# kivicode/TensorHive-Fixed

Hardware: AMD Instinct MI355X
Metric: llama3_8b_bf16_ddp_train_tokens_per_sec (higher is better)
Workload: dtype bf16; 1 GPU; model=Llama-3-8B, global_batch=8, micro_batch=8, grad_accum=1, seq_len=4096, parallelism=dp1, optimizer=AdamW (fp32 master, fused flat kernel, clip 1.0), zero=0, attention=hip, gemm_table=True, gemm_table_kind=gemm_gfx950_t32768.csv

## Files before the change

### tensorhive_fixed_amd/ops/csrc/flash_attn.hip

```cpp
#include "th_common.h"

typedef __bf16 bf16x8 __attribute__((ext_vector_type(8)));
typedef float f32x16 __attribute__((ext_vector_type(16)));
typedef short i16x4 __attribute__((ext_vector_type(4)));
#define LDS_AS __attribute__((address_space(3)))

namespace {
constexpr int HD = 128;
constexpr float LOG2E = 1.4426950408889634f;
constexpr float LN2 = 0.6931471805599453f;

__device__ __forceinline__ int img_off(int row, int ch) {
  return ((row >> 3) << 11) + ((ch >> 2) << 9) + ((row & 7) << 6) + (((ch & 3) ^ ((row >> 2) & 3)) << 4);
}

__device__ __forceinline__ bf16x8 as_bf(ushort8 u) { return __builtin_bit_cast(bf16x8, u); }

__device__ __forceinline__ bf16x8 lds_row(const char* img, int row, int ch) {
  return *reinterpret_cast<const bf16x8*>(img + img_off(row, ch));
}

__device__ __forceinline__ bf16x8 lds_tr(const char* img, int rbase, int cbase, int lane) {
  const int h = lane >> 5, grp = (lane >> 4) & 1, i = lane & 15;
  const int row = rbase + 4 * h + (i >> 2);
  const int col = cbase + 16 * grp + 4 * (i & 3);
  const char* p0 = img + img_off(row, col >> 3) + ((col & 7) << 1);
  const char* p1 = img + img_off(row + 8, col >> 3) + ((col & 7) << 1);
  const i16x4 lo = __builtin_amdgcn_ds_read_tr16_b64_v4i16((LDS_AS i16x4*)(p0));
  const i16x4 hi = __builtin_amdgcn_ds_read_tr16_b64_v4i16((LDS_AS i16x4*)(p1));
  typedef short i16x8 __attribute__((ext_vector_type(8)));
  const i16x8 v = {lo[0], lo[1], lo[2], lo[3], hi[0], hi[1], hi[2], hi[3]};
  return __builtin_bit_cast(bf16x8, v);
}

#ifndef TH_FA_PRIO
#define TH_FA_PRIO 1
#endif
#define FA_PRIO(p)                                  \
  do {                                              \
    if (TH_FA_PRIO) __builtin_amdgcn_s_setprio(p); \
  } while (0)

__device__ __forceinline__ f32x16 mfma(bf16x8 a, bf16x8 b, f32x16 c) {
  return __builtin_amdgcn_mfma_f32_32x32x16_bf16(a, b, c, 0, 0, 0);
}

__device__ __forceinline__ bf16x8 pack8(const f32x16& x, int base) {
  bf16x8 r;
#pragma unroll
  for (int j = 0; j < 8; ++j) r[j] = (__bf16)x[base + j];
  return r;
}

__device__ __forceinline__ void store_row_t21(ushort* row, const f32x16 (&acc)[4], float f, int h) {
#pragma unroll
  for (int d = 0; d < 4; ++d)
#pragma unroll
    for (int p = 0; p < 2; ++p) {
      unsigned a[2], c[2];
#pragma unroll
      for (int k = 0; k < 2; ++k) {
        a[k] = (unsigned)f2bf(acc[d][8 * p + 2 * k] * f) | ((unsigned)f2bf(acc[d][8 * p + 2 * k + 1] * f) << 16);
        c[k] = (unsigned)f2bf(acc[d][8 * p + 4 + 2 * k] * f) | ((unsigned)f2bf(acc[d][8 * p + 5 + 2 * k] * f) << 16);
        const auto r = __builtin_amdgcn_permlane32_swap(a[k], c[k], false, false);
        a[k] = r[0];
        c[k] = r[1];
      }
      typedef unsigned u32x4 __attribute__((ext_vector_type(4)));
      const u32x4 v = {a[0], a[1], c[0], c[1]};
      *reinterpret_cast<u32x4*>(row + 32 * d + 16 * p + 8 * h) = v;
    }
}

__device__ __forceinline__ void rope_bwd_rows(f32x16 (&a)[4], const float* __restrict__ rcos,
                                              const float* __restrict__ rsin, int pos, int h) {
  const float* cr = rcos + (long)pos * 64;
  const float* sr = rsin + (long)pos * 64;
#pragma unroll
  for (int d = 0; d < 2; ++d)
#pragma unroll
    for (int g = 0; g < 4; ++g) {
      const float4v c4 = *reinterpret_cast<const float4v*>(cr + 32 * d + 8 * g + 4 * h);
      const float4v s4 = *reinterpret_cast<const float4v*>(sr + 32 * d + 8 * g + 4 * h);
#pragma unroll
      for (int e = 0; e < 4; ++e) {
        const float x = a[d][4 * g + e], y = a[d + 2][4 * g + e];
        a[d][4 * g + e] = x * c4[e] + y * s4[e];
        a[d + 2][4 * g + e] = y * c4[e] - x * s4[e];
      }
    }
}

__device__ __forceinline__ int xcd_remap(int bid, int nwg) {
  const int xcd = bid & 7, q = nwg >> 3, r = nwg & 7;
  return (xcd < r ? xcd * (q + 1) : r * (q + 1) + (xcd - r) * q) + (bid >> 3);
}

__device__ __forceinline__ int acc_row(int r, int h) { return (r & 3) + 8 * (r >> 2) + 4 * h; }

__device__ __forceinline__ int stage_row(int tid) { return 2 * ((tid >> 3) & 7) + ((tid >> 2) & 1); }
__device__ __forceinline__ int stage_ch(int tid) { return 4 * ((tid >> 6) & 3) + (tid & 3); }
template <int NP>
__device__ __forceinline__ void stage_load(ushort8 (&r)[NP], const ushort* base, long ld, int row0,
                                           int limit, int tid) {
#pragma unroll
  for (int i = 0; i < NP; ++i) {
    const int row = min(row0 + 16 * i + stage_row(tid), limit - 1);
    r[i] = *reinterpret_cast<const ushort8*>(base + (long)row * ld + (stage_ch(tid) << 3));
  }
}
template <int NP>
__device__ __forceinline__ void stage_store(char* img, const ushort8 (&r)[NP], int tid) {
#pragma unroll
  for (int i = 0; i < NP; ++i)
    *reinterpret_cast<ushort8*>(img + img_off(16 * i + stage_row(tid), stage_ch(tid))) = r[i];
}

template <bool KVMAJOR>
__device__ __forceinline__ void q_block_map(int L, int nqb, int B, int Hq, int Hkv, int& b, int& hq, int& qb) {
  if (KVMAJOR) {
    const int G = Hq / Hkv, per = nqb * G;
    const int grp = L / per, r = L % per;
    b = grp / Hkv;
    hq = (grp % Hkv) * G + r % G;
    qb = nqb - 1 - r / G;
  } else {
    const int per = Hq * B;
    qb = nqb - 1 - L / per;
    const int rem = L % per;
    b = rem / Hq;
    hq = rem % Hq;
  }
}

__device__ __forceinline__ void glds16(const void* sbase, unsigned voff, unsigned lds) {
  asm volatile("s_mov_b32 m0, %0\n\ts_nop 0\n\tglobal_load_lds_dwordx4 %1, %2"
               :: "s"(lds), "v"(voff), "s"(sbase) : "memory", "m0");
}
__device__ __forceinline__ void glds4(const void* sbase, unsigned voff, unsigned lds) {
  asm volatile("s_mov_b32 m0, %0\n\ts_nop 0\n\tglobal_load_lds_dword %1, %2"
               :: "s"(lds), "v"(voff), "s"(sbase) : "memory", "m0");
}
__device__ __forceinline__ unsigned img_rc(unsigned o) {
  const unsigned row = ((o >> 11) << 3) | ((o >> 6) & 7);
  const unsigned ch = (((o >> 9) & 3) << 2) | (((o >> 4) & 3) ^ ((row >> 2) & 3));
  return row | (ch << 8);
}
__device__ __forceinline__ void wait_dma_barrier() { asm volatile("s_waitcnt vmcnt(0)\n\ts_barrier" ::: "memory"); }
__device__ __forceinline__ void dma_kv_tile(const ushort* Kb, const ushort* Vb, long ld, int S, int jt, unsigned lds0,
                                            int wu, const unsigned (&rc)[4]) {
  const unsigned img = lds0 + (jt & 1) * (2 * 64 * 256) + wu * 4096;
#pragma unroll
  for (int u = 0; u < 4; ++u) {
    const int row = min(jt * 64 + (int)(rc[u] & 255), S - 1);
    const unsigned voff = (unsigned)(row * ld + (rc[u] >> 8) * 8) * 2u;
    glds16(Kb, voff, img + u * 1024);
    glds16(Vb, voff, img + 64 * 256 + u * 1024);
  }
}

__device__ __forceinline__ void dma_kv_piece(const ushort* Kb, const ushort* Vb, long ld, int S, int jt,
                                             unsigned lds0, int wu, const unsigned (&rc)[4], int p) {
  const unsigned img = lds0 + (jt & 1) * (2 * 64 * 256) + wu * 4096;
  const int u = p >> 1;
  const int row = min(jt * 64 + (int)(rc[u] & 255), S - 1);
  const unsigned voff = (unsigned)(row * ld + (rc[u] >> 8) * 8) * 2u;
  if (p & 1)
    glds16(Vb, voff, img + 64 * 256 + u * 1024);
  else
    glds16(Kb, voff, img + u * 1024);
}

#ifndef TH_FA_FWD_SPREAD
#define TH_FA_FWD_SPREAD 0
#endif
#ifndef TH_FA_FWD_DEFAULT
#define TH_FA_FWD_DEFAULT 15
#endif
// ... 218 lines not shown
          if (ks4 == 2) {
            pf[2] = pack8(sacc[1], 0);
            pf[3] = pack8(sacc[1], 8);
          }
          bf16x8 nx[4];
#pragma unroll
          for (int d = 0; d < 4; ++d) nx[d] = ks4 < 3 ? lds_tr(vs, 16 * ks4 + 16, 32 * d, lane) : vt[d];
          __builtin_amdgcn_sched_barrier(0);
#pragma unroll
          for (int d = 0; d < 4; ++d) {
            o[d] = mfma(vt[d], pf[ks4], o[d]);
            if (ks4 < 2) {
              p_of(1, 8 * ks4 + 2 * d);
              p_of(1, 8 * ks4 + 2 * d + 1);
            }
          }
          __builtin_amdgcn_sched_barrier(0);
#pragma unroll
          for (int d = 0; d < 4; ++d) vt[d] = nx[d];
        }
        FA_PRIO(0);
      }
      const float rs = (rs4[0] + rs4[1]) + (rs4[2] + rs4[3]);
      l_i += half_swap_sum(rs);
    }
  }

  if (q < S) {
    const float inv_l = l_i > 0.f ? 1.f / l_i : 0.f;
    store_row_t21(O + b * bso + (long)q * ldo + (long)hq * HD, o, inv_l, h);
    if (h == 0) LSE[((long)b * Hq + hq) * S + q] = (m_i + log2f(l_i)) * LN2;
  }
}

#ifdef TH_FA_DIAG
constexpr int PP_R = 4, PP_SLOT = 2 * F_BN * 256;
#ifndef TH_PP_PRIO
#define TH_PP_PRIO 0
#endif
#ifndef TH_PP_SHIFT
#define TH_PP_SHIFT 0
#endif
#ifndef TH_PP_NMF
#define TH_PP_NMF 0
#endif
#ifndef TH_PP_YPRIO
#define TH_PP_YPRIO 0
#endif
#ifdef TH_PP_STAMP
constexpr int PP_STAMP_STEPS = 72;
__device__ unsigned long long th_pp_stamp_buf[8 * PP_STAMP_STEPS * 5];
#define PP_STAMP(i, k)                                                                                  \
  do {                                                                                                  \
    if (blockIdx.x == 0 && lane == 0 && (i) < PP_STAMP_STEPS)                                           \
      stamp_lds[(wu * PP_STAMP_STEPS + (i)) * 5 + (k)] = __builtin_amdgcn_s_memtime();                  \
  } while (0)
#else
#define PP_STAMP(i, k) \
  do {                 \
  } while (0)
#endif

__device__ __forceinline__ bool pp_has(int wu, int u, int T) { return wu < 4 ? u < T : (u >= 1 && u <= T); }
__device__ __forceinline__ void pp_wait(int wu, int need, int last, int part, int T) {
  if (need > T) return;
  int n = 0;
// ... 222 lines not shown
  }
  if (!half) pp_barrier();
#ifdef TH_PP_STAMP
  if (blockIdx.x == 0) {
    __syncthreads();
    for (int t = tid; t < 8 * PP_STAMP_STEPS * 5; t += 512) th_pp_stamp_buf[t] = stamp_lds[t];
  }
#endif

  if (q < S) {
    const float inv_l = l_i > 0.f ? 1.f / l_i : 0.f;
    store_row_t21(O + b * bso + (long)q * ldo + (long)hq * HD, o, inv_l, h);
    if (h == 0) LSE[((long)b * Hq + hq) * S + q] = (m_i + log2f(l_i)) * LN2;
  }
}
#endif

#ifndef TH_DQ_PRIO_ON
#define TH_DQ_PRIO_ON 1
#endif
#define TH_DQ_PRIO(p)                                     \
  do {                                                    \
    if (TH_DQ_PRIO_ON) __builtin_amdgcn_s_setprio(p);    \
  } while (0)
#ifndef TH_DQ_AHEAD
#define TH_DQ_AHEAD 1
#endif
#ifndef TH_DQ_PREKB
#define TH_DQ_PREKB 1
#endif
#ifndef TH_DQ_TR_AHEAD
#define TH_DQ_TR_AHEAD 1
#endif
template <bool KVMAJOR, bool DMA, bool SPREAD = false, bool L2OUT = false>
__global__ __launch_bounds__(256, 2) void fa_bwd_dq_kernel(
    const ushort* __restrict__ Q, const ushort* __restrict__ K, const ushort* __restrict__ V,
    const ushort* __restrict__ dO, const ushort* __restrict__ O, const float* __restrict__ LSE,
    float* __restrict__ Dl, ushort* __restrict__ dQ, int B, int S, int Hq, int Hkv, long ld, long bs, long ldo,
    long bso, float scale, float scale_log2, int causal, const float* __restrict__ rcos,
    const float* __restrict__ rsin) {
  __shared__ __attribute__((aligned(1024))) char smem_dq[(DMA ? 2 : 1) * 2 * F_BN * 256];
  const int nqb = (S + F_BM - 1) / F_BM;
  const int L = xcd_remap(blockIdx.x, gridDim.x);
  int b, hq, qb;
  q_block_map<KVMAJOR>(L, nqb, B, Hq, Hkv, b, hq, qb);
  const int hk = hq / (Hq / Hkv);
  const int tid = threadIdx.x, lane = tid & 63, w = tid >> 6, h = lane >> 5, c32 = lane & 31;
  const int q0 = qb * F_BM + w * 32;
  const int q = q0 + c32;
  const ushort* Qb = Q + b * bs + (long)hq * HD;
  const ushort* Kb = K + b * bs + (long)hk * HD;
  const ushort* Vb = V + b * bs + (long)hk * HD;
  const ushort* dOb = dO + b * bso + (long)hq * HD;
  const ushort* Ob = O + b * bso + (long)hq * HD;

  bf16x8 qf[8], gf[8];
  ushort8 qraw[8];
  float dpart = 0.f;
#pragma unroll
  for (int s = 0; s < 8; ++s) {
    qraw[s] = q < S ? *reinterpret_cast<const ushort8*>(Qb + (long)q * ld + 16 * s + 8 * h) : ushort8(0);
    const ushort8 graw = q < S ? *reinterpret_cast<const ushort8*>(dOb + (long)q * ldo + 16 * s + 8 * h) : ushort8(0);
    const ushort8 oraw = q < S ? *reinterpret_cast<const ushort8*>(Ob + (long)q * ldo + 16 * s + 8 * h) : ushort8(0);
    gf[s] = as_bf(graw);
#pragma unroll
    for (int e = 0; e < 8; ++e) dpart += bf2f(oraw[e]) * bf2f(graw[e]);
  }
  const long st = ((long)b * Hq + hq) * S;
// ... 145 lines not shown
          if (TH_DQ_PREKB && DMA && kb == 0 && d == 2) {
#pragma unroll
            for (int s = 0; s < 2; ++s) {
              pka[s] = lds_row(ks, 32 + c32, 2 * s + h);
              pva[s] = lds_row(vs, 32 + c32, 2 * s + h);
            }
          }
          __builtin_amdgcn_sched_barrier(0);
          dq[d] = mfma(t0, s0, dq[d]);
          dq[d] = mfma(t1, s1, dq[d]);
          __builtin_amdgcn_sched_barrier(0);
          t0 = n0;
          t1 = n1;
        }
        TH_DQ_PRIO(0);
      }
#endif
#else
#pragma unroll
      for (int d = 0; d < 4; ++d) {
        dq[d] = mfma(lds_tr(ks, 32 * kb, 32 * d, lane), s0, dq[d]);
        dq[d] = mfma(lds_tr(ks, 32 * kb + 16, 32 * d, lane), s1, dq[d]);
      }
#endif
    }
  }
  if (q < S) {
    if (rcos != nullptr) {
      rope_bwd_rows(dq, rcos, rsin, q, h);
    }
    store_row_t21(dQ + b * bs + (long)q * ld + (long)hq * HD, dq, scale, h);
  }
}

constexpr int B_BK = 256, B_BQ = 32, B_THREADS = 512;

template <bool KVMAJOR>
__global__ __launch_bounds__(B_THREADS, 2) void fa_bwd_dkv_kernel(
    const ushort* __restrict__ Q, const ushort* __restrict__ K, const ushort* __restrict__ V,
    const ushort* __restrict__ dO, const float* __restrict__ LSE, const float* __restrict__ Dl,
    ushort* __restrict__ dK, ushort* __restrict__ dV, int B, int S, int Hq, int Hkv, long ld,
    long bs, long ldo, long bso, float scale, float scale_log2, int causal, int young_prio) {
  extern __shared__ __attribute__((aligned(16))) char smem[];
  char* ks = smem;
  char* vs = ks + B_BK * 256;
  char* qs = vs + B_BK * 256;
  char* gs = qs + B_BQ * 256;
  float* ls = reinterpret_cast<float*>(gs + B_BQ * 256);
  float* ds = ls + B_BQ;
  const int nkb = (S + B_BK - 1) / B_BK;
  const int L = xcd_remap(blockIdx.x, gridDim.x);
  int b, hk, kblk;
  if (KVMAJOR) {
    const int grp = L / nkb, r = L % nkb;
    b = grp / Hkv;
    hk = grp % Hkv;
    kblk = causal ? r : nkb - 1 - r;
  } else {
    const int per = Hkv * B;
    kblk = causal ? L / per : nkb - 1 - L / per;
    const int rem = L % per;
    b = rem / Hkv;
    hk = rem % Hkv;
  }
  const int G = Hq / Hkv;
  const int tid = threadIdx.x, lane = tid & 63, w = tid >> 6, h = lane >> 5, c32 = lane & 31;
// ... 739 lines not shown
                  rsin, smem, b, hk, (causal ? kb_i : nkb - 1 - kb_i) * KF_BK);
  }
}

constexpr int B_LDS = 2 * B_BK * 256 + 2 * B_BQ * 256 + 2 * B_BQ * 4;
}

static int check_geom(int B, int S, int Hq, int Hkv, int D, long ld, long ldo) {
  if (B <= 0 || S <= 0 || Hq <= 0 || Hkv <= 0 || Hq % Hkv != 0 || D != HD) return -1;
  if (ld % 8 != 0 || ldo % 8 != 0) return -1;
  return 0;
}

extern "C" int th_flash_attn_fwd(const void* q, const void* k, const void* v, void* o, float* lse,
                                 int B, int S, int Hq, int Hkv, int D, int causal, long ld, long bs,
                                 long ldo, long bso, float scale, int flags, hipStream_t s) {
  if (check_geom(B, S, Hq, Hkv, D, ld, ldo)) return -1;
  const long nblk = (long)((S + F_BM - 1) / F_BM) * Hq * B;
  if (flags & 64) {
#ifdef TH_FA_DIAG
    if ((Hq / Hkv) % 2 != 0 || (long)S * ld * 2 >= (1L << 31)) return -3;
    const long npp = (long)((S + F_BM - 1) / F_BM) * (Hq / 2) * B;
    fa_fwd_pp_kernel<<<(unsigned)npp, 512, 0, s>>>((const ushort*)q, (const ushort*)k, (const ushort*)v,
                                                    (ushort*)o, lse, B, S, Hq, Hkv, ld, bs, ldo, bso,
                                                    scale * LOG2E, causal);
    TH_CHECK_LAUNCH();
#else
    return -3;
#endif
  }
  int var = flags >= 16 ? (flags & 15) : TH_FA_FWD_DEFAULT;
  bool spread = flags >= 16 ? ((flags >> 5) & 1) : TH_FA_FWD_SPREAD;
  if ((long)S * ld * 2 >= (1L << 31)) var &= ~4;
#define TH_FWD(P, Dd, Db, Km)                                                                      \
  fa_fwd_kernel<P, Dd, Db, Km><<<(unsigned)nblk, 256, 0, s>>>((const ushort*)q, (const ushort*)k,  \
                                                             (const ushort*)v, (ushort*)o, lse, B,  \
                                                             S, Hq, Hkv, ld, bs, ldo, bso,          \
                                                             scale * LOG2E, causal)
#ifdef TH_FA_DIAG
  if (var == 15 && spread) {
    fa_fwd_kernel<true, true, true, true, true><<<(unsigned)nblk, 256, 0, s>>>(
        (const ushort*)q, (const ushort*)k, (const ushort*)v, (ushort*)o, lse, B, S, Hq, Hkv, ld, bs, ldo, bso,
        scale * LOG2E, causal);
    TH_CHECK_LAUNCH();
  }
  switch (var) {
    case 0: TH_FWD(false, false, false, false); break;
    case 1: TH_FWD(true, false, false, false); break;
    case 2: TH_FWD(false, true, false, false); break;
    case 3: TH_FWD(true, true, false, false); break;
    case 4: TH_FWD(false, false, true, false); break;
    case 5: TH_FWD(true, false, true, false); break;
    case 6: TH_FWD(false, true, true, false); break;
    case 7: TH_FWD(true, true, true, false); break;
    case 8: TH_FWD(false, false, false, true); break;
    case 11: TH_FWD(true, true, false, true); break;
    case 15: TH_FWD(true, true, true, true); break;
    default: TH_FWD(true, true, true, true); break;
  }
#else
  if (spread || (var != 15 && var != 11)) return -3;
  if (var == 15) TH_FWD(true, true, true, true);
  else TH_FWD(true, true, false, true);
#endif
#undef TH_FWD
  TH_CHECK_LAUNCH();
}

#ifdef TH_PP_STAMP
extern "C" int th_pp_stamps(void* dst) {
  return (int)hipMemcpyFromSymbol(dst, HIP_SYMBOL(th_pp_stamp_buf), sizeof(th_pp_stamp_buf));
}
#endif

static int kf_var_of(int flags) { return (flags >> 6) & 8191; }
static bool kf_variant_known(int v) {
  return v == 7535
#ifdef TH_FA_DIAG
         || v == 0 || v == 111 || v == 3439
#endif
#ifdef TH_KF_DIAG
         || v == 3567 || v == 7663
#endif
      ;
}

static bool flags_shipped(int flags) {
#ifdef TH_FA_DIAG
  (void)flags;
  return true;
#else
  const int known = 8 | 16 | 32 | (8191 << 6) | (1 << 19);
  if (flags & ~known) return false;
  if (flags & 32) return !(flags & 16);
  if (!((flags >> 19) & 1)) return false;
  if (flags & 16) return !(flags & 8) && kf_variant_known(kf_var_of(flags));
  return kf_var_of(flags) == 0;
#endif
}

static int flash_bwd_impl(const void* q, const void* k, const void* v, const void* o, const void* dout,
                          const float* lse, float* delta, void* dq, void* dk, void* dv, int B, int S, int Hq,
                          int Hkv, int D, int causal, long ld, long bs, long ldo, long bso, float scale,
                          const float* rcos, const float* rsin, int flags, hipStream_t s) {
  if (check_geom(B, S, Hq, Hkv, D, ld, ldo)) return -1;
  if (rcos != nullptr && ((flags & (8 | 32)) || (long)S * ld * 2 >= (1L << 31) || rsin == nullptr))
    return -3;
  if ((flags & 16) && !kf_variant_known(kf_var_of(flags))) return -3;
  if (!flags_shipped(flags)) return -3;
  if ((flags & 16) && S % C_BQ != 0) flags &= ~16;
  const long nq = (long)((S + F_BM - 1) / F_BM) * Hq * B;
  const bool dq_dma = !(flags & 32) && (long)S * ld * 2 < (1L << 31);
  const bool dq_spread = (flags >> 19) & 1;
  const bool dq_l2 = (flags & 16) && !(flags & 8) && dq_dma && (kf_var_of(flags) & 4096);
  if (dq_l2 && !(dq_spread && !(flags & 1))) return -3;
  if (dq_l2) {
    fa_bwd_dq_kernel<true, true, true, true><<<(unsigned)nq, 256, 0, s>>>(
        (const ushort*)q, (const ushort*)k, (const ushort*)v, (const ushort*)dout, (const ushort*)o, lse, delta,
        (ushort*)dq, B, S, Hq, Hkv, ld, bs, ldo, bso, scale, scale * LOG2E, causal, rcos, rsin);
  } else {
#define TH_DQ_LAUNCH(KVM, DMA_, SP_)                                                                         \
  fa_bwd_dq_kernel<KVM, DMA_, SP_><<<(unsigned)nq, 256, 0, s>>>((const ushort*)q, (const ushort*)k, (const ushort*)v, \
                                                               (const ushort*)dout, (const ushort*)o, lse, delta,     \
                                                               (ushort*)dq, B, S, Hq, Hkv, ld, bs, ldo, bso, scale,   \
                                                               scale * LOG2E, causal, rcos, rsin)
#ifdef TH_FA_DIAG
  if (flags & 1) {
    if (dq_dma) {
      if (dq_spread) TH_DQ_LAUNCH(false, true, true); else TH_DQ_LAUNCH(false, true, false);
    } else {
      TH_DQ_LAUNCH(false, false, false);
    }
  } else {
    if (dq_dma) {
      if (dq_spread) TH_DQ_LAUNCH(true, true, true); else TH_DQ_LAUNCH(true, true, false);
    } else {
      TH_DQ_LAUNCH(true, false, false);
    }
  }
#else
  if (dq_dma) TH_DQ_LAUNCH(true, true, true);
  else TH_DQ_LAUNCH(true, false, false);
#endif
#undef TH_DQ_LAUNCH
  }
  if ((flags & 16) && !(flags & 8) && dq_dma) {
    const int kvar = kf_var_of(flags);
    const int nkb_f = (S + KF_BK - 1) / KF_BK;
    const long nkf = (long)((kvar & 32) ? (nkb_f + 1) / 2 : nkb_f) * Hkv * B;
#define TH_KF_LAUNCH(V_)                                                                                      \
  fa_bwd_kf_kernel<V_><<<(unsigned)nkf, 256, 0, s>>>((const ushort*)q, (const ushort*)k, (const ushort*)v,        \
                                                     (const ushort*)dout, lse, delta, (ushort*)dk, (ushort*)dv,   \
                                                     B, S, Hq, Hkv, ld, bs, ldo, bso, scale, scale * LOG2E, causal, \
                                                     rcos, rsin)
    switch (kvar) {
#ifdef TH_FA_DIAG
      case 0: TH_KF_LAUNCH(0); break;
      case 111: TH_KF_LAUNCH(111); break;
      case 3439: TH_KF_LAUNCH(3439); break;
#endif
      case 7535: TH_KF_LAUNCH(7535); break;
#ifdef TH_KF_DIAG
      case 3567: TH_KF_LAUNCH(3567); break;
      case 7663: TH_KF_LAUNCH(7663); break;
#endif
      default: return -3;
    }
#undef TH_KF_LAUNCH
    TH_CHECK_LAUNCH();
  }
  if (!(flags & 8) && dq_dma) {
    const long nkh = (long)((S + KH_BK - 1) / KH_BK) * Hkv * B;
    fa_bwd_kh_kernel<<<(unsigned)nkh, 256, 0, s>>>((const ushort*)q, (const ushort*)k, (const ushort*)v,
                                                   (const ushort*)dout, lse, delta, (ushort*)dk, (ushort*)dv,
                                                   B, S, Hq, Hkv, ld, bs, ldo, bso, scale, scale * LOG2E, causal,
                                                   rcos, rsin);
    TH_CHECK_LAUNCH();
  }
// ... 51 lines not shown
```

Before: 26840 tokens/s.

## Rewrite flash-attention dQ backward on 16x16x32 MFMA with new LDS swizzle

Replaces the shipped dQ backward kernel with a version built on 16x16x32 bf16 MFMA instructions, using a new LDS swizzle, transposed-read helpers and permlane-based row reductions and stores. The old 32x32x16 dQ kernel is kept only under the diagnostic build, and a 16x16 forward kernel is added behind a diagnostic flag. The aim is better MFMA and LDS scheduling in the dQ pass, with smaller accumulator tiles and possibly fewer registers. In exchange it brings a large new code path with its own layout and reduction logic that must stay numerically equivalent.

```diff
diff --git a/tensorhive_fixed_amd/ops/csrc/flash_attn.hip b/tensorhive_fixed_amd/ops/csrc/flash_attn.hip
--- a/tensorhive_fixed_amd/ops/csrc/flash_attn.hip
+++ b/tensorhive_fixed_amd/ops/csrc/flash_attn.hip
@@ -2,6 +2,7 @@
 
 typedef __bf16 bf16x8 __attribute__((ext_vector_type(8)));
 typedef float f32x16 __attribute__((ext_vector_type(16)));
+typedef float f32x4 __attribute__((ext_vector_type(4)));
 typedef short i16x4 __attribute__((ext_vector_type(4)));
 #define LDS_AS __attribute__((address_space(3)))
 
@@ -33,6 +34,42 @@
   return __builtin_bit_cast(bf16x8, v);
 }
 
+__device__ __forceinline__ int img_swz16(int row) { return ((((row >> 2) ^ (row >> 3)) & 1) << 1) | ((row >> 3) & 1); }
+__device__ __forceinline__ int img_off16(int row, int ch) {
+  return ((row >> 3) << 11) + ((ch >> 2) << 9) + ((row & 7) << 6) + (((ch & 3) ^ img_swz16(row)) << 4);
+}
+
+__device__ __forceinline__ bf16x8 lds_row16(const char* img, int row, int ch) {
+  return *reinterpret_cast<const bf16x8*>(img + img_off16(row, ch));
+}
+
+__device__ __forceinline__ bf16x8 lds_tr16(const char* img, int rbase, int cbase, int lane) {
+  const int g = lane >> 4, i = lane & 15;
+  const int row = rbase + 4 * g + (i >> 2);
+  const int col = cbase + 4 * (i & 3);
+  const char* p0 = img + img_off16(row, col >> 3) + ((col & 7) << 1);
+  const char* p1 = img + img_off16(row + 16, col >> 3) + ((col & 7) << 1);
+  const i16x4 lo = __builtin_amdgcn_ds_read_tr16_b64_v4i16((LDS_AS i16x4*)(p0));
+  const i16x4 hi = __builtin_amdgcn_ds_read_tr16_b64_v4i16((LDS_AS i16x4*)(p1));
+  typedef short i16x8 __attribute__((ext_vector_type(8)));
+  const i16x8 v = {lo[0], lo[1], lo[2], lo[3], hi[0], hi[1], hi[2], hi[3]};
+  return __builtin_bit_cast(bf16x8, v);
+}
+
+__device__ __forceinline__ f32x4 mfma16(bf16x8 a, bf16x8 b, f32x4 c) {
+  return __builtin_amdgcn_mfma_f32_16x16x32_bf16(a, b, c, 0, 0, 0);
+}
+
+__device__ __forceinline__ bf16x8 pack2x4(const f32x4& lo, const f32x4& hi) {
+  bf16x8 r;
+#pragma unroll
+  for (int j = 0; j < 4; ++j) {
+    r[j] = (__bf16)lo[j];
+    r[4 + j] = (__bf16)hi[j];
+  }
+  return r;
+}
+
 #ifndef TH_FA_PRIO
 #define TH_FA_PRIO 1
 #endif
@@ -91,6 +128,47 @@
     }
 }
 
+__device__ __forceinline__ float row_swap_sum(float x) {
+  const int xi = __builtin_bit_cast(int, x);
+  const auto r = __builtin_amdgcn_permlane16_swap(xi, xi, false, false);
+  return __builtin_bit_cast(float, (int)r[0]) + __builtin_bit_cast(float, (int)r[1]);
+}
+
+__device__ __forceinline__ void store_row16(ushort* row, const f32x4 (&acc)[8], float f, int g) {
+#pragma unroll
+  for (int t = 0; t < 4; ++t) {
+    unsigned a[2], c[2];
+#pragma unroll
+    for (int k = 0; k < 2; ++k) {
+      a[k] = (unsigned)f2bf(acc[2 * t][2 * k] * f) | ((unsigned)f2bf(acc[2 * t][2 * k + 1] * f) << 16);
+      c[k] = (unsigned)f2bf(acc[2 * t + 1][2 * k] * f) | ((unsigned)f2bf(acc[2 * t + 1][2 * k + 1] * f) << 16);
+      const auto r = __builtin_amdgcn_permlane16_swap(a[k], c[k], false, false);
+      a[k] = r[0];
+      c[k] = r[1];
+    }
+    typedef unsigned u32x4 __attribute__((ext_vector_type(4)));
+    const u32x4 v = {a[0], a[1], c[0], c[1]};
+    *reinterpret_cast<u32x4*>(row + 32 * t + 16 * (g & 1) + 8 * (g >> 1)) = v;
+  }
+}
+
+__device__ __forceinline__ void rope_bwd_rows16(f32x4 (&a)[8], const float* __restrict__ rcos,
+                                                const float* __restrict__ rsin, int pos, int g) {
+  const float* cr = rcos + (long)pos * 64;
+  const float* sr = rsin + (long)pos * 64;
+#pragma unroll
+  for (int d = 0; d < 4; ++d) {
+    const float4v c4 = *reinterpret_cast<const float4v*>(cr + 16 * d + 4 * g);
+    const float4v s4 = *reinterpret_cast<const float4v*>(sr + 16 * d + 4 * g);
+#pragma unroll
+    for (int e = 0; e < 4; ++e) {
+      const float x = a[d][e], y = a[d + 4][e];
+      a[d][e] = x * c4[e] + y * s4[e];
+      a[d + 4][e] = y * c4[e] - x * s4[e];
+    }
+  }
+}
+
 __device__ __forceinline__ int xcd_remap(int bid, int nwg) {
   const int xcd = bid & 7, q = nwg >> 3, r = nwg & 7;
   return (xcd < r ? xcd * (q + 1) : r * (q + 1) + (xcd - r) * q) + (bid >> 3);
@@ -114,6 +192,13 @@
 #pragma unroll
   for (int i = 0; i < NP; ++i)
     *reinterpret_cast<ushort8*>(img + img_off(16 * i + stage_row(tid), stage_ch(tid))) = r[i];
+}
+
+template <int NP>
+__device__ __forceinline__ void stage_store16(char* img, const ushort8 (&r)[NP], int tid) {
+#pragma unroll
+  for (int i = 0; i < NP; ++i)
+    *reinterpret_cast<ushort8*>(img + img_off16(16 * i + stage_row(tid), stage_ch(tid))) = r[i];
 }
 
 template <bool KVMAJOR>
@@ -144,6 +229,11 @@
 __device__ __forceinline__ unsigned img_rc(unsigned o) {
   const unsigned row = ((o >> 11) << 3) | ((o >> 6) & 7);
   const unsigned ch = (((o >> 9) & 3) << 2) | (((o >> 4) & 3) ^ ((row >> 2) & 3));
+  return row | (ch << 8);
+}
+__device__ __forceinline__ unsigned img_rc16(unsigned o) {
+  const unsigned row = ((o >> 11) << 3) | ((o >> 6) & 7);
+  const unsigned ch = (((o >> 9) & 3) << 2) | (((o >> 4) & 3) ^ (unsigned)img_swz16((int)row));
   return row | (ch << 8);
 }
 __device__ __forceinline__ void wait_dma_barrier() { asm volatile("s_waitcnt vmcnt(0)\n\ts_barrier" ::: "memory"); }
@@ -428,6 +518,220 @@
     if (h == 0) LSE[((long)b * Hq + hq) * S + q] = (m_i + log2f(l_i)) * LN2;
   }
 }
+
+#ifdef TH_FA_DIAG
+__device__ __forceinline__ void quad_max2(float& a, float& b) {
+  auto r = __builtin_amdgcn_permlane16_swap(__builtin_bit_cast(int, a), __builtin_bit_cast(int, b), false, false);
+  const float x = half_swap_max(fmaxf(__builtin_bit_cast(float, (int)r[0]), __builtin_bit_cast(float, (int)r[1])));
+  r = __builtin_amdgcn_permlane16_swap(__builtin_bit_cast(int, x), __builtin_bit_cast(int, x), false, false);
+  a = __builtin_bit_cast(float, (int)r[0]);
+  b = __builtin_bit_cast(float, (int)r[1]);
+}
+
+template <bool PRESCALE, bool DEFER, bool DBUF, bool KVMAJOR, bool SPREAD = false>
+__global__ __launch_bounds__(256, 2) void fa16_fwd_kernel(
+    const ushort* __restrict__ Q, const ushort* __restrict__ K, const ushort* __restrict__ V,
+    ushort* __restrict__ O, float* __restrict__ LSE, int B, int S, int Hq, int Hkv, long ld,
+    long bs, long ldo, long bso, float scale_log2, int causal) {
+  static_assert(PRESCALE && DEFER, "the 16x16x32 forward implements the shipped PRESCALE + DEFER variants only");
+  constexpr int NBUF = DBUF ? 2 : 1;
+  __shared__ __attribute__((aligned(16))) char smem[NBUF * 2 * F_BN * 256];
+  const int nqb = (S + F_BM - 1) / F_BM;
+  const int L = xcd_remap(blockIdx.x, gridDim.x);
+  int b, hq, qb;
+  q_block_map<KVMAJOR>(L, nqb, B, Hq, Hkv, b, hq, qb);
+  const int hk = hq / (Hq / Hkv);
+  const int tid = threadIdx.x, lane = tid & 63, w = tid >> 6, g = lane >> 4, c = lane & 15;
+  const int q0 = qb * F_BM + w * 32;
+  const int qi[2] = {q0 + c, q0 + 16 + c};
+  const ushort* Qb = Q + b * bs + (long)hq * HD;
+  const ushort* Kb = K + b * bs + (long)hk * HD;
+  const ushort* Vb = V + b * bs + (long)hk * HD;
+
+  bf16x8 qf[2][4];
+#pragma unroll
+  for (int n = 0; n < 2; ++n)
+#pragma unroll
+    for (int s = 0; s < 4; ++s) {
+      ushort8 u = qi[n] < S ? *reinterpret_cast<const ushort8*>(Qb + (long)qi[n] * ld + 32 * s + 8 * g) : ushort8(0);
+#pragma unroll
+      for (int e = 0; e < 8; ++e) u[e] = f2bf(bf2f(u[e]) * scale_log2);
+      qf[n][s] = as_bf(u);
+    }
+
+  const int kv_end = causal ? min(S, qb * F_BM + F_BM) : S;
+  const int ntiles = (kv_end + F_BN - 1) / F_BN;
+  ushort8 kr[4], vr[4];
+  unsigned rc[4];
+  const unsigned lds0 = (unsigned)(uintptr_t)(char LDS_AS*)smem;
+  const int wu = __builtin_amdgcn_readfirstlane(w);
+  if (DBUF) {
+    __builtin_amdgcn_s_waitcnt(0x0F70);
+#pragma unroll
+    for (int u = 0; u < 4; ++u) rc[u] = img_rc16(w * 4096 + u * 1024 + lane * 16);
+    dma_kv_tile(Kb, Vb, ld, S, 0, lds0, wu, rc);
+  } else {
+    stage_load<4>(kr, Kb, ld, 0, S, tid);
+    stage_load<4>(vr, Vb, ld, 0, S, tid);
+  }
+
+  f32x4 o[2][8];
+#pragma unroll
+  for (int n = 0; n < 2; ++n)
+#pragma unroll
+    for (int d = 0; d < 8; ++d) o[n][d] = f32x4(0.f);
+  float m_i[2] = {-INFINITY, -INFINITY}, l_p[2] = {0.f, 0.f}, m_base[2] = {0.f, 0.f};
+  f32x4 s_init[2] = {f32x4(0.f), f32x4(0.f)};
+
+  for (int j = 0; j < ntiles; ++j) {
+    char* ks = smem + (DBUF ? (j & 1) : 0) * (2 * F_BN * 256);
+    char* vs = ks + F_BN * 256;
+    if (DBUF) {
+      wait_dma_barrier();
+      if (!SPREAD && j + 1 < ntiles) dma_kv_tile(Kb, Vb, ld, S, j + 1, lds0, wu, rc);
+    } else {
+      __syncthreads();
+      stage_store16<4>(ks, kr, tid);
+      stage_store16<4>(vs, vr, tid);
+      __syncthreads();
+      if (j + 1 < ntiles) {
+        stage_load<4>(kr, Kb, ld, (j + 1) * F_BN, S, tid);
+        stage_load<4>(vr, Vb, ld, (j + 1) * F_BN, S, tid);
+      }
+    }
+    const int kbase = j * F_BN;
+    const int jd = min(j + 1, ntiles - 1);
+    if (SPREAD && causal && kbase > q0 + 31) dma_kv_tile(Kb, Vb, ld, S, jd, lds0, wu, rc);
+    if (!(causal && kbase > q0 + 31)) {
+      f32x4 sacc[4][2];
+#pragma unroll
+      for (int n = 0; n < 4; ++n) {
+        sacc[n][0] = s_init[0];
+        sacc[n][1] = s_init[1];
+      }
+      {
+        FA_PRIO(1);
+        bf16x8 ka[3][2];
+#pragma unroll
+        for (int t = 0; t < 2; ++t) {
+          ka[t][0] = lds_row16(ks, 16 * (t >> 1) + c, 8 * (t & 1) + g);
+          ka[t][1] = lds_row16(ks, 16 * (t >> 1) + c, 8 * (t & 1) + 4 + g);
+          __builtin_amdgcn_sched_barrier(0);
+        }
+#pragma unroll
+        for (int u = 0; u < 8; ++u) {
+          if (u + 2 < 8) {
+            ka[(u + 2) % 3][0] = lds_row16(ks, 16 * ((u + 2) >> 1) + c, 8 * (u & 1) + g);
+            ka[(u + 2) % 3][1] = lds_row16(ks, 16 * ((u + 2) >> 1) + c, 8 * (u & 1) + 4 + g);
+          }
+          __builtin_amdgcn_sched_barrier(0);
+          const int n = u >> 1, s0 = 2 * (u & 1);
+          sacc[n][0] = mfma16(ka[u % 3][0], qf[0][s0], sacc[n][0]);
+          sacc[n][1] = mfma16(ka[u % 3][0], qf[1][s0], sacc[n][1]);
+          if (SPREAD) dma_kv_piece(Kb, Vb, ld, S, jd, lds0, wu, rc, u);
+          sacc[n][0] = mfma16(ka[u % 3][1], qf[0][s0 + 1], sacc[n][0]);
+          sacc[n][1] = mfma16(ka[u % 3][1], qf[1][s0 + 1], sacc[n][1]);
+          __builtin_amdgcn_sched_barrier(0);
+        }
+        FA_PRIO(0);
+      }
+      const bool need_mask = (causal && kbase + F_BN - 1 > q0) || (kbase + F_BN > S);
+      if (need_mask) {
+#pragma unroll
+        for (int qn = 0; qn < 2; ++qn) {
+          const int kmax = (causal ? min(qi[qn], S - 1) : S - 1) - kbase - 4 * g;
+#pragma unroll
+          for (int n = 0; n < 4; ++n)
+#pragma unroll
+            for (int i = 0; i < 4; ++i) sacc[n][qn][i] = (16 * n + i <= kmax) ? sacc[n][qn][i] : -INFINITY;
+        }
+      }
+      float mt[2] = {-INFINITY, -INFINITY};
+#pragma unroll
+      for (int qn = 0; qn < 2; ++qn)
+#pragma unroll
+        for (int n = 0; n < 4; ++n)
+#pragma unroll
+          for (int i = 0; i < 4; ++i) mt[qn] = fmaxf(mt[qn], sacc[n][qn][i]);
+      quad_max2(mt[0], mt[1]);
+      if (!__all(mt[0] + m_base[0] - m_i[0] <= F_DEFER_THR && mt[1] + m_base[1] - m_i[1] <= F_DEFER_THR)) {
+#pragma unroll
+        for (int qn = 0; qn < 2; ++qn) {
+          const float m_new = fmaxf(m_i[qn], mt[qn] + m_base[qn]);
+          const float mu = m_new == -INFINITY ? 0.f : m_new;
+          const float alpha = fast_exp2(m_i[qn] - mu);
+          l_p[qn] *= alpha;
+#pragma unroll
+          for (int d = 0; d < 8; ++d) o[qn][d] *= alpha;
+          m_i[qn] = m_new;
+          const float shift = mu - m_base[qn];
+#pragma unroll
+          for (int n = 0; n < 4; ++n) sacc[n][qn] -= shift;
+          m_base[qn] = mu;
+          s_init[qn] = f32x4(-mu);
+        }
+      }
+      float rs[2][2] = {{0.f, 0.f}, {0.f, 0.f}};
+      auto p_of = [&](int n, int qn, int i) {
+        const float p = fast_exp2(sacc[n][qn][i]);
+        sacc[n][qn][i] = p;
+        rs[qn][i & 1] += p;
+      };
+#pragma unroll
+      for (int n = 0; n < 2; ++n)
+#pragma unroll
+        for (int qn = 0; qn < 2; ++qn)
+#pragma unroll
+          for (int i = 0; i < 4; ++i) p_of(n, qn, i);
+      bf16x8 pf[2][2];
+      pf[0][0] = pack2x4(sacc[0][0], sacc[1][0]);
+      pf[0][1] = pack2x4(sacc[0][1], sacc[1][1]);
+      {
+        FA_PRIO(1);
+        bf16x8 vt[4];
+#pragma unroll
+        for (int d = 0; d < 4; ++d) vt[d] = lds_tr16(vs, 0, 16 * d, lane);
+#pragma unroll
+        for (int v = 0; v < 4; ++v) {
+          if (v == 2) {
+            pf[1][0] = pack2x4(sacc[2][0], sacc[3][0]);
+            pf[1][1] = pack2x4(sacc[2][1], sacc[3][1]);
+          }
+          bf16x8 nx[4];
+#pragma unroll
+          for (int d = 0; d < 4; ++d)
+            nx[d] = v < 3 ? lds_tr16(vs, 32 * ((v + 1) >> 1), 64 * ((v + 1) & 1) + 16 * d, lane) : vt[d];
+          __builtin_amdgcn_sched_barrier(0);
+#pragma unroll
+          for (int d = 0; d < 4; ++d) {
+            const int db = 4 * (v & 1) + d, e = 8 * v + 2 * d;
+            o[0][db] = mfma16(vt[d], pf[v >> 1][0], o[0][db]);
+            if (v < 2) p_of(2 + (e >> 3), (e >> 2) & 1, e & 3);
+            o[1][db] = mfma16(vt[d], pf[v >> 1][1], o[1][db]);
+            if (v < 2) p_of(2 + ((e + 1) >> 3), ((e + 1) >> 2) & 1, (e + 1) & 3);
+          }
+          __builtin_amdgcn_sched_barrier(0);
+#pragma unroll
+          for (int d = 0; d < 4; ++d) vt[d] = nx[d];
+        }
+        FA_PRIO(0);
+      }
+      l_p[0] += rs[0][0] + rs[0][1];
+      l_p[1] += rs[1][0] + rs[1][1];
+    }
+  }
+
+#pragma unroll
+  for (int qn = 0; qn < 2; ++qn) {
+    const float l_i = half_swap_sum(row_swap_sum(l_p[qn]));
+    if (qi[qn] < S) {
+      const float inv_l = l_i > 0.f ? 1.f / l_i : 0.f;
+      store_row16(O + b * bso + (long)qi[qn] * ldo + (long)hq * HD, o[qn], inv_l, g);
+      if (g == 0) LSE[((long)b * Hq + hq) * S + qi[qn]] = (m_i[qn] + log2f(l_i)) * LN2;
+    }
+  }
+}
+#endif
 
 #ifdef TH_FA_DIAG
 constexpr int PP_R = 4, PP_SLOT = 2 * F_BN * 256;
@@ -716,8 +1020,218 @@
 #ifndef TH_DQ_TR_AHEAD
 #define TH_DQ_TR_AHEAD 1
 #endif
+#if !defined(TH_FA_DIAG) && (TH_DQ_AHEAD != 1 || TH_DQ_TR_AHEAD != 1)
+#error "fa_bwd_dq_kernel implements TH_DQ_AHEAD=1 with TH_DQ_TR_AHEAD=1 only (the knobs steer the TH_FA_DIAG 32x32x16 body)"
+#endif
+#if TH_DQ_PREKB != 0 && TH_DQ_PREKB != 1
+#error "TH_DQ_PREKB is 0 or 1"
+#endif
 template <bool KVMAJOR, bool DMA, bool SPREAD = false, bool L2OUT = false>
 __global__ __launch_bounds__(256, 2) void fa_bwd_dq_kernel(
+    const ushort* __restrict__ Q, const ushort* __restrict__ K, const ushort* __restrict__ V,
+    const ushort* __restrict__ dO, const ushort* __restrict__ O, const float* __restrict__ LSE,
+    float* __restrict__ Dl, ushort* __restrict__ dQ, int B, int S, int Hq, int Hkv, long ld, long bs, long ldo,
+    long bso, float scale, float scale_log2, int causal, const float* __restrict__ rcos,
+    const float* __restrict__ rsin) {
+  __shared__ __attribute__((aligned(1024))) char smem_dq[(DMA ? 2 : 1) * 2 * F_BN * 256];
+  const int nqb = (S + F_BM - 1) / F_BM;
+  const int L = xcd_remap(blockIdx.x, gridDim.x);
+  int b, hq, qb;
+  q_block_map<KVMAJOR>(L, nqb, B, Hq, Hkv, b, hq, qb);
+  const int hk = hq / (Hq / Hkv);
+  const int tid = threadIdx.x, lane = tid & 63, w = tid >> 6, g = lane >> 4, c = lane & 15;
+  const int q0 = qb * F_BM + w * 32;
+  const int qi[2] = {q0 + c, q0 + 16 + c};
+  const ushort* Qb = Q + b * bs + (long)hq * HD;
+  const ushort* Kb = K + b * bs + (long)hk * HD;
+  const ushort* Vb = V + b * bs + (long)hk * HD;
+  const ushort* dOb = dO + b * bso + (long)hq * HD;
+  const ushort* Ob = O + b * bso + (long)hq * HD;
+  const long st = ((long)b * Hq + hq) * S;
+
+  bf16x8 qf[2][4], gf[2][4];
+  f32x4 s_init[2], p_init[2];
+#pragma unroll
+  for (int n = 0; n < 2; ++n) {
+    const int q = qi[n];
+    float dpart = 0.f;
+#pragma unroll
+    for (int s = 0; s < 4; ++s) {
+      ushort8 qraw = q < S ? *reinterpret_cast<const ushort8*>(Qb + (long)q * ld + 32 * s + 8 * g) : ushort8(0);
+      const ushort8 graw = q < S ? *reinterpret_cast<const ushort8*>(dOb + (long)q * ldo + 32 * s + 8 * g) : ushort8(0);
+      const ushort8 oraw = q < S ? *reinterpret_cast<const ushort8*>(Ob + (long)q * ldo + 32 * s + 8 * g) : ushort8(0);
+      gf[n][s] = as_bf(graw);
+#pragma unroll
+      for (int e = 0; e < 8; ++e) {
+        dpart += bf2f(oraw[e]) * bf2f(graw[e]);
+        qraw[e] = f2bf(bf2f(qraw[e]) * scale_log2);
+      }
+      qf[n][s] = as_bf(qraw);
+    }
+    const float lse2 = q < S ? LSE[st + q] * LOG2E : INFINITY;
+    const float dsum = half_swap_sum(row_swap_sum(dpart));
+    if (q < S && g == 0) Dl[st + q] = dsum;
+    if (L2OUT && q < S && g == 0) Dl[(long)B * Hq * S + st + q] = -lse2;
+    s_init[n] = f32x4(-lse2);
+    p_init[n] = f32x4(q < S ? -dsum : 0.f);
+  }
+
+  const int kv_end = causal ? min(S, qb * F_BM + F_BM) : S;
+  const int ntiles = (kv_end + F_BN - 1) / F_BN;
+  ushort8 kr[4], vr[4];
+  unsigned rc[4];
+  const unsigned lds0 = (unsigned)(uintptr_t)(char LDS_AS*)smem_dq;
+  const int wu = __builtin_amdgcn_readfirstlane(w);
+  auto dma_tile = [&](int jt) { dma_kv_tile(Kb, Vb, ld, S, jt, lds0, wu, rc); };
+  if (DMA) {
+    __builtin_amdgcn_s_waitcnt(0x0F70);
+#pragma unroll
+    for (int u = 0; u < 4; ++u) rc[u] = img_rc16(w * 4096 + u * 1024 + lane * 16);
+    dma_tile(0);
+  } else {
+    stage_load<4>(kr, Kb, ld, 0, S, tid);
+    stage_load<4>(vr, Vb, ld, 0, S, tid);
+  }
+  f32x4 dq[2][8];
+#pragma unroll
+  for (int n = 0; n < 2; ++n)
+#pragma unroll
+    for (int d = 0; d < 8; ++d) dq[n][d] = f32x4(0.f);
+
+  for (int j = 0; j < ntiles; ++j) {
+    char* ks = smem_dq + (DMA ? (j & 1) * (2 * F_BN * 256) : 0);
+    char* vs = ks + F_BN * 256;
+    if (DMA) {
+      wait_dma_barrier();
+      if (!SPREAD && j + 1 < ntiles) dma_tile(j + 1);
+    } else {
+      __syncthreads();
+      stage_store16<4>(ks, kr, tid);
+      stage_store16<4>(vs, vr, tid);
+      __syncthreads();
+      if (j + 1 < ntiles) {
+        stage_load<4>(kr, Kb, ld, (j + 1) * F_BN, S, tid);
+        stage_load<4>(vr, Vb, ld, (j + 1) * F_BN, S, tid);
+      }
+    }
+    const int kbase = j * F_BN;
+    const int jd = min(j + 1, ntiles - 1);
+    if (causal && kbase > q0 + 31) {
+      if (SPREAD) dma_tile(jd);
+      continue;
+    }
+    const bool need_mask = (causal && kbase + F_BN - 1 > q0) || (kbase + F_BN > S);
+    constexpr bool PREKB = TH_DQ_PREKB && DMA;
+    bf16x8 pka[2], pva[2];
+#pragma unroll
+    for (int kb = 0; kb < 2; ++kb) {
+      f32x4 sacc[2][2], pacc[2][2];
+#pragma unroll
+      for (int n = 0; n < 2; ++n)
+#pragma unroll
+        for (int qn = 0; qn < 2; ++qn) {
+          sacc[n][qn] = s_init[qn];
+          pacc[n][qn] = p_init[qn];
+        }
+      {
+        bf16x8 ka[2], va[2];
+#pragma unroll
+        for (int t = 0; t < 2; ++t) {
+          if (PREKB && kb == 1) {
+            ka[t] = pka[t];
+            va[t] = pva[t];
+          } else {
+            ka[t] = lds_row16(ks, 32 * kb + c, 4 * t + g);
+            va[t] = lds_row16(vs, 32 * kb + c, 4 * t + g);
+          }
+        }
+        TH_DQ_PRIO(1);
+#pragma unroll
+        for (int t = 0; t < 8; ++t) {
+          bf16x8 kn = ka[t & 1], vn = va[t & 1];
+          if (t + 2 < 8) {
+            kn = lds_row16(ks, 32 * kb + 16 * ((t + 2) >> 2) + c, 4 * ((t + 2) & 3) + g);
+            vn = lds_row16(vs, 32 * kb + 16 * ((t + 2) >> 2) + c, 4 * ((t + 2) & 3) + g);
+          }
+          __builtin_amdgcn_sched_barrier(0);
+          const int n = t >> 2, s = t & 3;
+          sacc[n][0] = mfma16(ka[t & 1], qf[0][s], sacc[n][0]);
+          sacc[n][1] = mfma16(ka[t & 1], qf[1][s], sacc[n][1]);
+          if (SPREAD && kb == 0) dma_kv_piece(Kb, Vb, ld, S, jd, lds0, wu, rc, t);
+          pacc[n][0] = mfma16(va[t & 1], gf[0][s], pacc[n][0]);
+          pacc[n][1] = mfma16(va[t & 1], gf[1][s], pacc[n][1]);
+          __builtin_amdgcn_sched_barrier(0);
+          ka[t & 1] = kn;
+          va[t & 1] = vn;
+        }
+        TH_DQ_PRIO(0);
+      }
+      if (need_mask) {
+#pragma unroll
+        for (int qn = 0; qn < 2; ++qn) {
+          const int kmax = (causal ? min(qi[qn], S - 1) : S - 1) - kbase - 32 * kb - 4 * g;
+#pragma unroll
+          for (int n = 0; n < 2; ++n)
+#pragma unroll
+            for (int i = 0; i < 4; ++i) {
+              float p = fast_exp2(sacc[n][qn][i]);
+              p = (16 * n + i <= kmax) ? p : 0.f;
+              sacc[n][qn][i] = p * pacc[n][qn][i];
+            }
+        }
+      } else {
+#pragma unroll
+        for (int qn = 0; qn < 2; ++qn)
+#pragma unroll
+          for (int n = 0; n < 2; ++n)
+#pragma unroll
+            for (int i = 0; i < 4; ++i) sacc[n][qn][i] = fast_exp2(sacc[n][qn][i]) * pacc[n][qn][i];
+      }
+      const bf16x8 ds0 = pack2x4(sacc[0][0], sacc[1][0]), ds1 = pack2x4(sacc[0][1], sacc[1][1]);
+      {
+        bf16x8 t0 = lds_tr16(ks, 32 * kb, 0, lane), t1 = lds_tr16(ks, 32 * kb, 16, lane);
+        TH_DQ_PRIO(1);
+#pragma unroll
+        for (int v = 0; v < 4; ++v) {
+          bf16x8 n0 = t0, n1 = t1;
+          if (v < 3) {
+            n0 = lds_tr16(ks, 32 * kb, 32 * v + 32, lane);
+            n1 = lds_tr16(ks, 32 * kb, 32 * v + 48, lane);
+          }
+          if (PREKB && kb == 0 && v == 2) {
+#pragma unroll
+            for (int t = 0; t < 2; ++t) {
+              pka[t] = lds_row16(ks, 32 + c, 4 * t + g);
+              pva[t] = lds_row16(vs, 32 + c, 4 * t + g);
+            }
+          }
+          __builtin_amdgcn_sched_barrier(0);
+          dq[0][2 * v] = mfma16(t0, ds0, dq[0][2 * v]);
+          dq[1][2 * v] = mfma16(t0, ds1, dq[1][2 * v]);
+          dq[0][2 * v + 1] = mfma16(t1, ds0, dq[0][2 * v + 1]);
+          dq[1][2 * v + 1] = mfma16(t1, ds1, dq[1][2 * v + 1]);
+          __builtin_amdgcn_sched_barrier(0);
+          t0 = n0;
+          t1 = n1;
+        }
+        TH_DQ_PRIO(0);
+      }
+    }
+  }
+#pragma unroll
+  for (int qn = 0; qn < 2; ++qn)
+    if (qi[qn] < S) {
+      if (rcos != nullptr) rope_bwd_rows16(dq[qn], rcos, rsin, qi[qn], g);
+      store_row16(dQ + b * bs + (long)qi[qn] * ld + (long)hq * HD, dq[qn], scale, g);
+    }
+}
+
+#ifdef TH_FA_DIAG
+#if TH_DQ_PREKB && !(TH_DQ_AHEAD && TH_DQ_TR_AHEAD == 1)
+#error "TH_DQ_PREKB fills its operands in the TH_DQ_AHEAD=1, TH_DQ_TR_AHEAD=1 dQ chain only: build with -DTH_DQ_PREKB=0"
+#endif
+template <bool KVMAJOR, bool DMA, bool SPREAD = false, bool L2OUT = false>
+__global__ __launch_bounds__(256, 2) void fa32_bwd_dq_kernel(
     const ushort* __restrict__ Q, const ushort* __restrict__ K, const ushort* __restrict__ V,
     const ushort* __restrict__ dO, const ushort* __restrict__ O, const float* __restrict__ LSE,
     float* __restrict__ Dl, ushort* __restrict__ dQ, int B, int S, int Hq, int Hkv, long ld, long bs, long ldo,
@@ -929,6 +1443,7 @@
     store_row_t21(dQ + b * bs + (long)q * ld + (long)hq * HD, dq, scale, h);
   }
 }
+#endif
 
 constexpr int B_BK = 256, B_BQ = 32, B_THREADS = 512;
 
@@ -1734,16 +2249,23 @@
   int var = flags >= 16 ? (flags & 15) : TH_FA_FWD_DEFAULT;
   bool spread = flags >= 16 ? ((flags >> 5) & 1) : TH_FA_FWD_SPREAD;
   if ((long)S * ld * 2 >= (1L << 31)) var &= ~4;
-#define TH_FWD(P, Dd, Db, Km)                                                                      \
-  fa_fwd_kernel<P, Dd, Db, Km><<<(unsigned)nblk, 256, 0, s>>>((const ushort*)q, (const ushort*)k,  \
-                                                             (const ushort*)v, (ushort*)o, lse, B,  \
-                                                             S, Hq, Hkv, ld, bs, ldo, bso,          \
-                                                             scale * LOG2E, causal)
+#define TH_FWD_K(KERN, P, Dd, Db, Km)                                                                \
+  KERN<P, Dd, Db, Km><<<(unsigned)nblk, 256, 0, s>>>((const ushort*)q, (const ushort*)k, (const ushort*)v, \
+                                                     (ushort*)o, lse, B, S, Hq, Hkv, ld, bs, ldo, bso,   \
+                                                     scale * LOG2E, causal)
+#define TH_FWD(P, Dd, Db, Km) TH_FWD_K(fa_fwd_kernel, P, Dd, Db, Km)
 #ifdef TH_FA_DIAG
+  const bool mfma16 = (flags & 128) != 0;
+  if (mfma16 && var != 15 && var != 11) return -3;
   if (var == 15 && spread) {
-    fa_fwd_kernel<true, true, true, true, true><<<(unsigned)nblk, 256, 0, s>>>(
-        (const ushort*)q, (const ushort*)k, (const ushort*)v, (ushort*)o, lse, B, S, Hq, Hkv, ld, bs, ldo, bso,
-        scale * LOG2E, causal);
+    if (mfma16)
+      fa16_fwd_kernel<true, true, true, true, true><<<(unsigned)nblk, 256, 0, s>>>(
+          (const ushort*)q, (const ushort*)k, (const ushort*)v, (ushort*)o, lse, B, S, Hq, Hkv, ld, bs, ldo, bso,
+          scale * LOG2E, causal);
+    else
+      fa_fwd_kernel<true, true, true, true, true><<<(unsigned)nblk, 256, 0, s>>>(
+          (const ushort*)q, (const ushort*)k, (const ushort*)v, (ushort*)o, lse, B, S, Hq, Hkv, ld, bs, ldo, bso,
+          scale * LOG2E, causal);
     TH_CHECK_LAUNCH();
   }
   switch (var) {
@@ -1756,15 +2278,22 @@
     case 6: TH_FWD(false, true, true, false); break;
     case 7: TH_FWD(true, true, true, false); break;
     case 8: TH_FWD(false, false, false, true); break;
-    case 11: TH_FWD(true, true, false, true); break;
-    case 15: TH_FWD(true, true, true, true); break;
+    case 11:
+      if (mfma16) TH_FWD_K(fa16_fwd_kernel, true, true, false, true);
+      else TH_FWD(true, true, false, true);
+      break;
+    case 15:
+      if (mfma16) TH_FWD_K(fa16_fwd_kernel, true, true, true, true);
+      else TH_FWD(true, true, true, true);
+      break;
     default: TH_FWD(true, true, true, true); break;
   }
 #else
-  if (spread || (var != 15 && var != 11)) return -3;
+  if (spread || (flags & 128) || (var != 15 && var != 11)) return -3;
   if (var == 15) TH_FWD(true, true, true, true);
   else TH_FWD(true, true, false, true);
 #endif
+#undef TH_FWD_K
 #undef TH_FWD
   TH_CHECK_LAUNCH();
 }
@@ -1816,16 +2345,24 @@
   const bool dq_spread = (flags >> 19) & 1;
   const bool dq_l2 = (flags & 16) && !(flags & 8) && dq_dma && (kf_var_of(flags) & 4096);
   if (dq_l2 && !(dq_spread && !(flags & 1))) return -3;
+#define TH_DQ_ARGS                                                                                                 \
+  (const ushort*)q, (const ushort*)k, (const ushort*)v, (const ushort*)dout, (const ushort*)o, lse, delta, (ushort*)dq, \
+      B, S, Hq, Hkv, ld, bs, ldo, bso, scale, scale * LOG2E, causal, rcos, rsin
+#ifdef TH_FA_DIAG
+  const bool dq_old32 = (flags >> 20) & 1;
+#define TH_DQ_LAUNCH(KVM, DMA_, SP_) fa32_bwd_dq_kernel<KVM, DMA_, SP_><<<(unsigned)nq, 256, 0, s>>>(TH_DQ_ARGS)
+#define TH_DQ16_LAUNCH(KVM, DMA_, SP_) fa_bwd_dq_kernel<KVM, DMA_, SP_><<<(unsigned)nq, 256, 0, s>>>(TH_DQ_ARGS)
+#else
+  const bool dq_old32 = false;
+#define TH_DQ_LAUNCH(KVM, DMA_, SP_) fa_bwd_dq_kernel<KVM, DMA_, SP_><<<(unsigned)nq, 256, 0, s>>>(TH_DQ_ARGS)
+#endif
   if (dq_l2) {
-    fa_bwd_dq_kernel<true, true, true, true><<<(unsigned)nq, 256, 0, s>>>(
-        (const ushort*)q, (const ushort*)k, (const ushort*)v, (const ushort*)dout, (const ushort*)o, lse, delta,
-        (ushort*)dq, B, S, Hq, Hkv, ld, bs, ldo, bso, scale, scale * LOG2E, causal, rcos, rsin);
+#ifdef TH_FA_DIAG
+    if (dq_old32) fa32_bwd_dq_kernel<true, true, true, true><<<(unsigned)nq, 256, 0, s>>>(TH_DQ_ARGS);
+    else
+#endif
+    fa_bwd_dq_kernel<true, true, true, true><<<(unsigned)nq, 256, 0, s>>>(TH_DQ_ARGS);
   } else {
-#define TH_DQ_LAUNCH(KVM, DMA_, SP_)                                                                         \
-  fa_bwd_dq_kernel<KVM, DMA_, SP_><<<(unsigned)nq, 256, 0, s>>>((const ushort*)q, (const ushort*)k, (const ushort*)v, \
-                                                               (const ushort*)dout, (const ushort*)o, lse, delta,     \
-                                                               (ushort*)dq, B, S, Hq, Hkv, ld, bs, ldo, bso, scale,   \
-                                                               scale * LOG2E, causal, rcos, rsin)
 #ifdef TH_FA_DIAG
   if (flags & 1) {
     if (dq_dma) {
@@ -1835,17 +2372,23 @@
     }
   } else {
     if (dq_dma) {
-      if (dq_spread) TH_DQ_LAUNCH(true, true, true); else TH_DQ_LAUNCH(true, true, false);
+      if (!dq_spread) TH_DQ_LAUNCH(true, true, false);
+      else if (dq_old32) TH_DQ_LAUNCH(true, true, true);
+      else TH_DQ16_LAUNCH(true, true, true);
     } else {
-      TH_DQ_LAUNCH(true, false, false);
+      if (dq_old32) TH_DQ_LAUNCH(true, false, false);
+      else TH_DQ16_LAUNCH(true, false, false);
     }
   }
 #else
   if (dq_dma) TH_DQ_LAUNCH(true, true, true);
   else TH_DQ_LAUNCH(true, false, false);
 #endif
+  }
 #undef TH_DQ_LAUNCH
-  }
+#undef TH_DQ16_LAUNCH
+#undef TH_DQ_ARGS
+  (void)dq_old32;
   if ((flags & 16) && !(flags & 8) && dq_dma) {
     const int kvar = kf_var_of(flags);
     const int nkb_f = (S + KF_BK - 1) / KF_BK;
```

Result: no change. 26910 tokens/s (median of 6 runs) (+0.3%).
